# Sreyan88/audio-ssl

Hardware: AMD Instinct MI355X
Metric: upstream clips/sec (1s@16kHz, 64-mel) (higher is better)
Workload: dtype bf16; 1 GPU; delores-m upstream step (log-mel + 2 views + q/k conv encoders + MoCo + 3 Barlow heads + bwd + SGD), 1 s @ 16 kHz, 64 mel, batch 512/GPU, queue 65536; global_batch=512, parallelism=dp1

## Files before the change

audio-ssl_amd/src/engine.py:

```python
import os

import torch

from src import _native as N

import os as _os
_STEM_VALU = _os.environ.get("AUDIOSSL_STEM_VALU") == "1"
BN_MOMENTUM = 0.1
BN_EPS = 1e-5
_BN_FUSED = _os.environ.get("AUDIOSSL_BN_FUSED", "1") != "0"


ONE_STREAM = os.environ.get("AUDIOSSL_ONE_STREAM", "0") == "1"


_CAPTURE_ORIGIN = []


class capture_scope:

    def __enter__(self):
        _CAPTURE_ORIGIN.append(torch.cuda.current_stream())
        return self

# ... 462 lines not shown
    arg = _empty((Nimg, d), torch.uint8, like=H2)
    N.call("maxmean_fwd", dtype, int(y.dtype == torch.float32), H2, y, arg, Nimg, T3, d)
    return y, arg


def maxmean_backward(dtype, dy, arg, H2):
    Nimg, T3, d = H2.shape
    dA2 = _empty((Nimg * T3, d), N.torch_dtype(dtype), like=H2)
    N.call("maxmean_bwd", dtype, GD, dy, arg, H2, dA2, Nimg, T3, d)
    return dA2


class ProjCtx:
    pass


def projector_forward(PP, Y, dtype, groups, B, update_running=True, Wc=None):
    kin = Y.shape[1]
    c = ProjCtx()
    c.dtype, c.B, c.groups, c.kin, c.y = dtype, B, groups, kin, Y
    W = Wc if Wc is not None else tuple(cast(dtype, PP[f"projector.{i}.weight"]) for i in (0, 3, 6))
    c.W = W
    D = W[0].shape[0]
    c.D = D
    M = groups * B

    def bn(a, prefix, affine, relu, out, adt=None):
        g = PP[prefix + ".weight"] if affine else None
        b = PP[prefix + ".bias"] if affine else None
        return bn_train_apply(dtype, ad if adt is None else adt, a, B, D, g, b, PP[prefix + ".running_mean"], PP[prefix + ".running_var"],
                              update_running, groups, relu, out)
    td = N.torch_dtype(dtype)
    ad = _ad(dtype)
    c.ad = ad
    o32 = int(ad == N.F32)
    c.cmean = None
    if dtype == N.BF16 and Y.dtype == torch.float32 and not HP and B <= 1024 and kin % 32 == 0 and SYNC_BN is None:
        c.y_hi, c.cmean = center_cast(Y, groups, B)
        c.y_lo = None
        c.a1 = linear_fwd(dtype, c.y_hi, W[0], M, D, kin, out_f32=o32)
    elif dtype == N.BF16 and Y.dtype == torch.float32:
        c.y_hi, c.y_lo = _empty((M, kin), td, like=Y), _empty((M, kin), td, like=Y)
        N.call("split_bf16", Y, c.y_hi, c.y_lo, M * kin)
        c.a1 = torch.zeros(M, D, dtype=torch.float32, device=Y.device)
        gemm(dtype, 0, 0, M, D, kin, c.y_hi, kin, W[0], kin, c.a1, D, out_f32=1, atomic=1)
        gemm(dtype, 0, 0, M, D, kin, c.y_lo, kin, W[0], kin, c.a1, D, out_f32=1, atomic=1)
    else:
        c.y_hi, c.y_lo = Y, None
        c.a1 = linear_fwd(dtype, Y, W[0], M, D, kin, out_f32=o32)
    c.ad1 = N.F32 if c.a1.dtype == torch.float32 else ad
    c.h1 = _empty((M, D), td, like=Y)
    c.st1 = bn(c.a1, "projector.1", True, 1, c.h1, adt=c.ad1)
    if c.cmean is not None and update_running:
        N.call("shift_running_mean", W[0], c.cmean, PP["projector.1.running_mean"], D, kin, groups, BN_MOMENTUM)
    c.a2 = linear_fwd(dtype, c.h1, W[1], M, D, D, out_f32=o32)
    c.h2 = _empty((M, D), td, like=Y)
    c.st2 = bn(c.a2, "projector.4", True, 1, c.h2)
    c.z = linear_fwd(dtype, c.h2, W[2], M, D, D, out_f32=o32)
    c.zn = _empty((M, D), td, like=Y)
    c.st0 = bn(c.z, "bn", False, 0, c.zn)
    return c.zn, c


def projector_backward(c, PP, G, dzn, dy_rows=None):
    dtype, B, D, kin, groups = c.dtype, c.B, c.D, c.kin, c.groups
    M = groups * B
    td = N.torch_dtype(dtype)

    def bn_bwd(a, dh, st, relu, da, g_gamma, g_beta, adt=None):
        adt = c.ad if adt is None else adt
        """BatchNorm1d(train) backward per group (view).  SyncBatchNorm (`extras/delores-s/main.py:79` converts every BatchNorm of
        the model, the projector's included): the two means of the backward are over the GLOBAL batch of the view - this rank's
        sums are all-reduced between the statistics pass and the apply pass; the parameter gradients stay this rank's own sums
        (the data-parallel gradient all-reduce adds the ranks up afterwards)."""
        t = ARENA.scratch((2 * groups * D,), torch.float64, dzn)
        if SYNC_BN is None:
            N.call("colbn_bwd", dtype, adt, GD, a, dh, *st, relu, groups, B, D, t, da, g_gamma, g_beta)
            return
        N.call("colbn_bwd_stats", dtype, adt, GD, a, dh, *st, relu, groups, B, D, t)
        tg = SYNC_BN.all_reduce(t.clone())
        N.call("colbn_bwd_apply", dtype, adt, GD, a, dh, *st, relu, groups, B, D, tg, float(B * SYNC_BN.world), da)
        if g_gamma is not None:
            for g in range(groups):
                N.call("add_d2f", t[g * D:(g + 1) * D], g_beta, D)
                N.call("add_d2f", t[(groups + g) * D:(groups + g + 1) * D], g_gamma, D)
    dz = _empty((M, D), td, like=c.zn)
    bn_bwd(c.z, dzn, c.st0, 0, dz, None, None)
    linear_bwd_w(dtype, dz, c.h2, G["projector.6.weight"], M, D, D)
    dh2 = linear_bwd_x(dtype, dz, c.W[2], M, D, D, out_f32=1)
    da2 = _empty((M, D), td, like=c.zn)
    bn_bwd(c.a2, dh2, c.st2, 1, da2, G["projector.4.weight"], G["projector.4.bias"])
    linear_bwd_w(dtype, da2, c.h1, G["projector.3.weight"], M, D, D)
    dh1 = linear_bwd_x(dtype, da2, c.W[1], M, D, D, out_f32=1)
    da1 = _empty((M, D), td, like=c.zn)
    bn_bwd(c.a1, dh1, c.st1, 1, da1, G["projector.1.weight"], G["projector.1.bias"], adt=c.ad1)
    linear_bwd_w(dtype, da1, c.y_hi, G["projector.0.weight"], M, D, kin)
    if c.y_lo is not None:
        linear_bwd_w(dtype, da1, c.y_lo, G["projector.0.weight"], M, D, kin)
    rows = M if dy_rows is None else dy_rows
    if rows == 0:
        return None
    return linear_bwd_x(dtype, da1, c.W[0], rows, D, kin, out_f32=1)


def barlow_forward_backward(PP, G, Y, dtype, lambd, scale_loss, loss_out, need_dy1=True, need_dy2=True,
                            update_running=True, all_reduce=None, global_batch=None, backward=True, Wc=None):
    B = Y.shape[0] // 2
    zn, c = projector_forward(PP, Y, dtype, 2, B, update_running, Wc)
    D = c.D
    zn1, zn2 = zn[:B], zn[B:]
    denom = float(global_batch if global_batch else B)
    cmat = _empty((D, D), torch.float32, like=Y)
    gemm(dtype, 1, 1, D, D, B, zn1, D, zn2, D, cmat, D, alpha=1.0 / denom, out_f32=1)
    if all_reduce is not None:
        all_reduce(cmat)
    coef = (lambd if lambd else 1.0) * scale_loss
    dc = _empty((D, D), N.torch_dtype(dtype), like=Y)
    N.call("barlow_loss", dtype, cmat, D, coef, 2.0 * coef / denom, dc, loss_out)
    if not backward:
        return None
    dzn = _empty((2 * B, D), torch.float32, like=Y)
    gemm(dtype, 0, 0, B, D, D, zn2, D, dc, D, dzn[:B], D, out_f32=1)
    gemm(dtype, 0, 1, B, D, D, zn1, D, dc, D, dzn[B:], D, out_f32=1)
    rows = 2 * B if need_dy2 else (B if need_dy1 else 0)
    return projector_backward(c, PP, G, dzn, rows)


def _harr(ctype, xs):
    import ctypes
    vals = [x.data_ptr() if isinstance(x, torch.Tensor) else x for x in xs]
    return (ctype * len(vals))(*vals)


def _multi_check(*lists):
    for ts in lists:
        for t in ts:
            if t is not None and (not t.is_cuda or not t.is_contiguous()):
                raise RuntimeError("multi-problem launches need contiguous device tensors")


def gemm_multi(ta, tb, M, Nn, Ks, As, ldas, Bs, ldbs, Cs, ldc, alpha=1.0, out_f32=0, atomic=0, ksplit=1):
    import ctypes
    n = len(As)
    _multi_check(As, Bs, Cs)
    Ns = [Nn] * n if isinstance(Nn, int) else list(Nn)
    ldcs = [ldc] * n if isinstance(ldc, int) else list(ldc)
    adr = ctypes.addressof
    arrs = (_harr(ctypes.c_int, Ns), _harr(ctypes.c_int, Ks), _harr(ctypes.c_void_p, As), _harr(ctypes.c_long, ldas),
            _harr(ctypes.c_void_p, Bs), _harr(ctypes.c_long, ldbs), _harr(ctypes.c_void_p, Cs), _harr(ctypes.c_long, ldcs))
    N_, K_, A_, la_, B_, lb_, C_, lc_ = arrs
    if N.PROFILE is not None:
        N.PROFILE_NOTE = float(sum(2.0 * M * nn * kk for nn, kk in zip(Ns, Ks)))
    N.call("gemm_multi", n, ta, tb, M, adr(N_), adr(K_), float(alpha), adr(A_), adr(la_), adr(B_), adr(lb_), adr(C_), adr(lc_),
           out_f32, atomic, ksplit)


def gemm_multi_sgd(ta, tb, M, Nn, Ks, As, ldas, Bs, ldbs, Ps, Moms, Shadows, ldp, hyper, alpha=1.0):
    import ctypes
    n = len(As)
    _multi_check(As, Bs, Ps, Moms, [] if Shadows is None else Shadows)
    Ns = [Nn] * n if isinstance(Nn, int) else list(Nn)
    ldps = [ldp] * n if isinstance(ldp, int) else list(ldp)
    adr = ctypes.addressof
    vp = ctypes.c_void_p
    arrs = (_harr(ctypes.c_int, Ns), _harr(ctypes.c_int, Ks), _harr(vp, As), _harr(ctypes.c_long, ldas), _harr(vp, Bs),
            _harr(ctypes.c_long, ldbs), _harr(vp, Ps), _harr(vp, Moms), _harr(vp, Shadows if Shadows is not None else [None] * n),
            _harr(ctypes.c_long, ldps))
    if N.PROFILE is not None:
        N.PROFILE_NOTE = (float(sum(2.0 * M * nn * kk for nn, kk in zip(Ns, Ks))),
                          float(sum(2.0 * kk * (M + nn) + M * nn * (16.0 + (2.0 if Shadows is not None else 0.0)) for nn, kk in zip(Ns, Ks))))
    lr, mu, wd, gs, gs_dev = hyper
    N.call("gemm_multi_sgd", n, ta, tb, M, adr(arrs[0]), adr(arrs[1]), float(alpha), adr(arrs[2]), adr(arrs[3]), adr(arrs[4]), adr(arrs[5]),
           adr(arrs[6]), adr(arrs[7]), adr(arrs[8]), adr(arrs[9]), float(lr), float(mu), float(wd), float(gs), gs_dev)


def _heads_wgrad_split(D, kmax, M, nh):
    return _ksplit(D, kmax, M, max(256 // nh, 1))


def heads_wgrads_store(D, kins, M, grads_zero=True):
    nh = len(kins)
    return bool(grads_zero) and all(_heads_wgrad_split(D, k, M, nh) == 1 for k in (D, max(kins)))


def barlow_heads_forward_backward(PPs, Gs, Ys, dtype, lambds, scale_losses, loss_outs, update_running=True, backward=True,
                                  Wcs=None, grads_zero=False, dy_ready=None, sgd=None):
    import ctypes
    nh = len(Ys)
    B = Ys[0].shape[0] // 2
    M = 2 * B
    td = N.torch_dtype(dtype)
    dev = Ys[0].device
    W = Wcs if Wcs is not None else [tuple(cast(dtype, PP[f"projector.{i}.weight"]) for i in (0, 3, 6)) for PP in PPs]
    D = W[0][0].shape[0]
    kins = [Y.shape[1] for Y in Ys]
    ad = _ad(dtype)
    if dtype != N.BF16 or ad != N.BF16 or B > 1024 or D % 32:
        raise RuntimeError("grouped Barlow heads: bf16 path with B <= 1024 only")
    H = range(nh)
    vp, fl, adr = ctypes.c_void_p, ctypes.c_float, ctypes.addressof
    new = lambda rows, cols, t: [torch.empty(rows, cols, dtype=t, device=dev) for _ in H]

    def layer(xs, ws, ks, prefix, affine, relu):
        a = new(M, D, td)
        gemm_multi(0, 0, M, D, ks, xs, ks, ws, ks, a, D)
        out, st = new(M, D, td), new(4, 2 * D, torch.float32)
        par = lambda suffix, on=True: _harr(vp, [PP[prefix + suffix] if on else None for PP in PPs])
        arrs = (_harr(vp, a), par(".weight", affine), par(".bias", affine), par(".running_mean", update_running),
                par(".running_var", update_running), _harr(vp, out), _harr(vp, st))
        _multi_check(a, out, st)
        N.call("colbn_train_fwd_multi", nh, ad, adr(arrs[0]), adr(arrs[1]), adr(arrs[2]), adr(arrs[3]), adr(arrs[4]),
               BN_MOMENTUM, BN_EPS, relu, 2, B, D, adr(arrs[5]), adr(arrs[6]))
        return a, st, out
    ycs = [torch.empty(M, k, dtype=torch.bfloat16, device=dev) for k in kins]
    cms = [torch.empty(2, k, dtype=torch.float32, device=dev) for k in kins]
    _multi_check(list(Ys), ycs, cms)
    if any(Y.dtype != torch.float32 or k % 32 for Y, k in zip(Ys, kins)):
        raise RuntimeError("grouped Barlow heads: fp32 inputs with width % 32 == 0")
    arrs = (_harr(vp, list(Ys)), _harr(vp, ycs), _harr(vp, cms), _harr(ctypes.c_int, kins))
    N.call("center_cast_multi", nh, adr(arrs[0]), adr(arrs[1]), adr(arrs[2]), adr(arrs[3]), 2, B)
    a1, st1, h1 = layer(ycs, [W[h][0] for h in H], kins, "projector.1", True, 1)

    def shift_running():
        rms = [PP["projector.1.running_mean"] for PP in PPs]
        w0 = [W[h][0] for h in H]
        _multi_check(w0, rms)
        arrs = (_harr(vp, w0), _harr(vp, cms), _harr(vp, rms), _harr(ctypes.c_int, kins))
        N.call("shift_running_mean_multi", nh, adr(arrs[0]), adr(arrs[1]), adr(arrs[2]), D, adr(arrs[3]), 2, BN_MOMENTUM)
    shift_late = update_running and backward and dy_ready is not None
    if update_running and not shift_late:
        shift_running()
    a2, st2, h2 = layer(h1, [W[h][1] for h in H], [D] * nh, "projector.4", True, 1)
    z, st0, zn = layer(h2, [W[h][2] for h in H], [D] * nh, "bn", False, 0)
    dc = new(D, D, td)
    coefs = [(lambds[h] if lambds[h] else 1.0) * scale_losses[h] for h in H]
    dsc = [2.0 * c / B for c in coefs]
    if all(l.numel() == LOSS_REPLICAS for l in loss_outs) and D % 64 == 0:
        _multi_check([zn[h] for h in H], dc, list(loss_outs))
        arrs = (_harr(ctypes.c_int, [B] * nh), _harr(vp, [zn[h][:B] for h in H]), _harr(ctypes.c_long, [D] * nh),
                _harr(vp, [zn[h][B:] for h in H]), _harr(ctypes.c_long, [D] * nh), _harr(vp, dc), _harr(fl, coefs), _harr(fl, dsc),
                _harr(vp, list(loss_outs)))
        if N.PROFILE is not None:
            N.PROFILE_NOTE = float(nh * 2.0 * D * D * B)
        N.call("gemm_multi_barlow", nh, D, adr(arrs[0]), 1.0 / B, adr(arrs[1]), adr(arrs[2]), adr(arrs[3]), adr(arrs[4]), adr(arrs[5]),
               adr(arrs[6]), adr(arrs[7]), adr(arrs[8]))
    else:
        cm = new(D, D, torch.float32)
        gemm_multi(1, 1, D, D, [B] * nh, [zn[h][:B] for h in H], [D] * nh, [zn[h][B:] for h in H], [D] * nh, cm, D,
                   alpha=1.0 / B, out_f32=1)
        arrs = (_harr(vp, cm), _harr(fl, coefs), _harr(fl, dsc), _harr(vp, dc), _harr(vp, list(loss_outs)))
        _multi_check(list(loss_outs))
        N.call("barlow_loss_multi", nh, adr(arrs[0]), D, adr(arrs[1]), adr(arrs[2]), adr(arrs[3]), adr(arrs[4]))
    if not backward:
        return [None] * nh
    dzn = new(M, D, torch.float32)
    gemm_multi(0, 0, B, D, [D] * nh, [zn[h][B:] for h in H], [D] * nh, dc, [D] * nh, [dzn[h][:B] for h in H], D, out_f32=1)
    gemm_multi(0, 1, B, D, [D] * nh, [zn[h][:B] for h in H], [D] * nh, dc, [D] * nh, [dzn[h][B:] for h in H], D, out_f32=1)

    def bn_bwd(a, dh, st, relu, names):
        out = new(M, D, td)
        grads = lambda k: _harr(vp, [Gs[h][names[k]] if names else None for h in H])
        arrs = (_harr(vp, a), _harr(vp, dh), _harr(vp, st), _harr(vp, out), grads(0), grads(1))
        _multi_check(a, dh, st)
        N.call("colbn_bwd_multi", nh, ad, GD, adr(arrs[0]), adr(arrs[1]), adr(arrs[2]), relu, 2, B, D, adr(arrs[3]),
               adr(arrs[4]), adr(arrs[5]))
        return out

    def wgrad(dys, xs, name, ks):
        split = _heads_wgrad_split(D, max(ks), M, nh)
        if sgd is not None:
            if split != 1 or Wcs is None:
                raise RuntimeError("fused SGD needs unsplit weight gradients and the flat weight shadows")
            li = {"projector.0.weight": 0, "projector.3.weight": 1, "projector.6.weight": 2}[name]
            gemm_multi_sgd(1, 1, D, ks, [M] * nh, dys, [D] * nh, xs, ks, [PPs[h][name] for h in H], [sgd["momentum"][h][name] for h in H],
                           [W[h][li] for h in H], ks, sgd["hyper"])
            return
        gemm_multi(1, 1, D, ks, [M] * nh, dys, [D] * nh, xs, ks, [Gs[h][name] for h in H], ks, out_f32=1,
                   atomic=1 if split > 1 else (0 if grads_zero else 2), ksplit=split)

    def dgrad(dys, ws, Ks, rows):
        out = [torch.empty(rows, k, dtype=torch.float32, device=dev) for k in Ks]
        gemm_multi(0, 1, rows, Ks, [D] * nh, [dy[:rows] for dy in dys], [D] * nh, ws, Ks, out, Ks, out_f32=1)
        return out
    later = []
    defer = (lambda fn: later.append(fn)) if dy_ready is not None else (lambda fn: fn())
    dz = bn_bwd(z, dzn, st0, 0, None)
    defer(lambda: wgrad(dz, h2, "projector.6.weight", [D] * nh))
    dh2 = dgrad(dz, [W[h][2] for h in H], [D] * nh, M)
    da2 = bn_bwd(a2, dh2, st2, 1, ("projector.4.weight", "projector.4.bias"))
    defer(lambda: wgrad(da2, h1, "projector.3.weight", [D] * nh))
    dh1 = dgrad(da2, [W[h][1] for h in H], [D] * nh, M)
    da1 = bn_bwd(a1, dh1, st1, 1, ("projector.1.weight", "projector.1.bias"))
    defer(lambda: wgrad(da1, ycs, "projector.0.weight", kins))
    dy = dgrad(da1, [W[h][0] for h in H], kins, B)
    if dy_ready is not None:
        dy_ready()
    if shift_late:
        shift_running()
    for fn in later:
        fn()
    return dy


def moco_forward_backward(dtype, q, k, queue, queue_shadow, temperature, loss_out, backward=True):
    B, dim = q.shape
    K = queue.shape[1]
    td = N.torch_dtype(dtype)
    qn, kn = _empty((B, dim), td, like=q), _empty((B, dim), td, like=q)
    qn32, kn32 = _empty((B, dim), torch.float32, like=q), _empty((B, dim), torch.float32, like=q)
    qinv, kinv = _empty((B,), torch.float32, like=q), _empty((B,), torch.float32, like=q)
    lpos = _empty((B,), torch.float32, like=q)
    N.call("moco_prep", dtype, q, k, B, dim, 1.0 / temperature, qn, qn32, qinv, kn, kn32, kinv, lpos)
    lse = _empty((B,), torch.float32, like=q)
    dlpos = _empty((B,), torch.float32, like=q)
    Pm = None
    if dtype == N.BF16 and K % 8 == 0 and dim % 8 == 0:
        nslot = (K + 63) // 64
        part = _empty((B, nslot, 2), torch.float32, like=q)
        N.call("moco_logits", 1, qn, queue_shadow, B, K, dim, 1.0 / temperature, part, None, 0.0, None)
        N.call("moco_lse_merge", lpos, part, B, nslot, 1.0 / (B * temperature), lse, loss_out, dlpos)
        if not backward:
            return None, kn32
        Pm = _empty((B, K), td, like=q)
        N.call("moco_logits", 2, qn, queue_shadow, B, K, dim, 1.0 / temperature, None, lse, 1.0 / (B * temperature), Pm)
    else:
        lneg = _empty((B, K), torch.float32, like=q)
        gemm(dtype, 0, 1, B, K, dim, qn, dim, queue_shadow, K, lneg, K, alpha=1.0 / temperature, out_f32=1)
        N.call("moco_ce_fwd", lpos, lneg, B, K, lse, loss_out)
        if not backward:
            return None, kn32
        Pm = _empty((B, K), td, like=q)
        N.call("moco_ce_bwd", dtype, lpos, lneg, lse, B, K, 1.0 / (B * temperature), Pm, dlpos)
    dqn = ARENA.zeros((B, dim), torch.float32, device=q.device)
    gemm(dtype, 0, 0, B, dim, K, Pm, K, queue_shadow, K, dqn, dim, out_f32=1, atomic=1, ksplit=_ksplit(B, dim, K, 256))
    dq = _empty((B, dim), td, like=q)
    N.call("l2norm_bwd", dtype, dqn, dlpos, kn32, qn32, qinv, B, dim, dq)
    return dq, kn32
```

include/audiossl_hip.h:

```cpp
#ifndef AUDIOSSL_HIP_H
#define AUDIOSSL_HIP_H

#include <stdint.h>

#ifdef __cplusplus
extern "C" {
#endif

#define AUDIOSSL_OK 0
#define AUDIOSSL_EINVAL (-1)
#define AUDIOSSL_ELAUNCH (-2)
#define AUDIOSSL_EALIGN (-3)

int audiossl_logmel_fwd(const float* wave, float* out, int B, int L, int T, int n_fft, int hop, int n_mels, int taps,
                        const float* win, const float* tw, const float* melw, const int* mel_start, float eps_pow,
                        float eps_log, int apply_log, void* stream);

int audiossl_clip_moments(const float* x, double* mom, int B, int n, void* stream);
int audiossl_runnorm_scan(const double* mom, int B, int n_elem, long long* state_i, float* state_f, float* mu_out,
                          float* sd_out, void* stream);
int audiossl_aug_normalize(const float* x, const float* mu, const float* sd, float* bank, long slot0, int R, int B, int n,
                           void* stream);
int audiossl_aug_views(const float* bank, int R, const int* ip, const float* fp, float* out1, float* out2, int B, int F,
                       int T, int canvas_h, int canvas_w, int log_mix, void* stream);
int audiossl_aug_plan_host(uint32_t* np_key, int* np_pos, uint32_t* py_key, int* py_pos, int B, int F, int T,
                           long long clips_seen, long long* n_entries, int R, int n_memory, int use_mix, double ratio,
                           int use_rrc, double fs_lo, double fs_hi, double ts_lo, double ts_hi, int canvas_h,
                           int canvas_w, int use_spec, int spec_F, int spec_T, int spec_nf, int spec_nt, const int* lens,
                           int unit, int* starts, int* ip, float* fp, int* masks);

int audiossl_resample_sinc(const float* x, float* y, int clips, int n_orig, int n_out, const int* n, const int* off_l,
                           const int* off_r, const double* eta_l, const double* eta_r, const double* win, const double* delta,
                           int nwin, int index_step, void* stream);

int audiossl_kmix_cluster(const float* views, const float* centroids, int n_views, int F, int T, int K, int* cluster,
                          void* stream);
int audiossl_kmix_apply(const float* views, const float* ring, const int* slot, const float* coef, int n_views, int n,
                        int log_mix, float* out, void* stream);
int audiossl_mask_fill(float* x, const int* tab, int n_img, int max_masks, int F, int T, int zero_fill, void* stream);

int audiossl_conv1_stats(const float* img, int N, int F, int T, const float* w, const float* bias, const float* gamma,
                         const float* beta, float* running_mean, float* running_var, float momentum, float eps,
                         double* mom, float* scale, float* shift, float* save_mean, float* save_rstd, void* stream);
#define AUDIOSSL_CONV1_XL_PARTS 4
int audiossl_conv1_fwd(int dtype, const float* img, int N, int F, int T, const float* w, const float* bias,
                       const float* scale, const float* shift, void* out, float* xl, void* stream);
int audiossl_conv1_bwd(int dtype, int conv_dtype, const float* img, int N, int F, int T, const float* w, const float* bias,
                       const float* gamma, const float* scale, const float* shift, const float* mean, const float* rstd,
                       const double* mom, const void* dP, const void* dxl, float* acc, float* dW, float* dbias,
                       float* dgamma, float* dbeta, void* stream);

int audiossl_colstats(int dtype, const void* x, int groups, long M, int C, long ld, int want_sq, double* sum,
                      double* sumsq, void* stream);
int audiossl_bn_finalize(const double* sum, const double* sumsq, int groups, double count, int C, const float* gamma,
                         const float* beta, float* running_mean, float* running_var, float momentum, float eps,
                         float* scale, float* shift, float* save_mean, float* save_rstd, void* stream);
int audiossl_bn_relu_pool_fwd(int dtype, int ydtype, const void* Y, const float* scale, const float* shift, void* P, int N,
                              int Ti, int Fi, void* stream);
int audiossl_bn_relu_pool_train_fwd(int dtype, int ydtype, const void* Y, const double* sum, const double* sumsq, int stat_replicas,
                                    double count, const float* gamma, const float* beta, float* running_mean, float* running_var,
                                    float momentum, float eps, void* P, float* scale, float* shift, float* save_mean, float* save_rstd,
                                    int N, int Ti, int Fi, void* stream);
int audiossl_tmean_fwd(int dtype, int out_f32, const void* P, void* xl, int N, int To, int Fo, void* stream);
int audiossl_tmean3_fwd(int dtype, int out_f32, const void* P1, void* x1, const float* x1_parts, int To1, int Fo1, const void* P2,
                        void* x2, int To2, int Fo2, const void* P3, void* x3, int To3, int Fo3, int N, void* stream);
int audiossl_bn_relu_pool_bwd(int dtype, int ydtype, int gdtype, const void* Y, const void* dP, const void* dxl, const float* scale,
                              const float* shift, const float* mean, const float* rstd, float* stat, void* dY,
                              float* dgamma, float* dbeta, int N, int Ti, int Fi, void* stream);
int audiossl_bn_relu_pool_bwd_p(int dtype, int ydtype, int gdtype, const void* Y, const void* P, const void* dP, const void* dxl,
                                const float* scale, const float* shift, const float* mean, const float* rstd, float* stat, void* dY,
                                float* dgamma, float* dbeta, int N, int Ti, int Fi, void* stream);
int audiossl_conv1_moments(const float* img, int N, int F, int T, double* mom, void* stream);
int audiossl_conv1_finalize(double* mom_totals, const float* w, const float* bias, const float* gamma, const float* beta,
                            float* running_mean, float* running_var, float momentum, float eps, double count, float* scale,
                            float* shift, float* save_mean, float* save_rstd, void* stream);
int audiossl_conv1_bwd_sums(int dtype, int conv_dtype, const float* img, int N, int F, int T, const float* w, const float* bias,
                            const float* gamma, const float* scale, const float* shift, const float* mean, const float* rstd,
                            const double* mom, const void* dP, const void* dxl, float* acc, float* lstat, void* stream);
int audiossl_conv1_bwd_finalize(const float* acc, const double* mom, const float* w, const float* bias, const float* gamma,
                                const float* mean, const float* rstd, double count_global, const float* gstat, float* dW,
                                float* dbias, float* dgamma, float* dbeta, void* stream);
int audiossl_bn_relu_pool_bwd_stats(int dtype, int ydtype, int gdtype, const void* Y, const void* dP, const void* dxl,
                                    const float* scale, const float* shift, const float* mean, const float* rstd, float* stat,
                                    int N, int Ti, int Fi, void* stream);
int audiossl_bn_relu_pool_bwd_apply(int dtype, int ydtype, int gdtype, const void* Y, const void* dP, const void* dxl,
                                    const float* scale, const float* shift, const float* mean, const float* rstd, float* stat,
                                    const float* gstat, double count_global, void* dY, float* dgamma, float* dbeta, int N, int Ti,
                                    int Fi, void* stream);
int audiossl_colbn_bwd_stats(int dtype, int adtype, int gdtype, const void* a, const void* dh, const float* scale,
                             const float* shift, const float* mean, const float* rstd, int relu, int groups, long M, int C,
                             double* tmp, void* stream);
int audiossl_colbn_bwd_apply(int dtype, int adtype, int gdtype, const void* a, const void* dh, const float* scale,
                             const float* shift, const float* mean, const float* rstd, int relu, int groups, long M, int C,
                             const double* sums, double count, void* da, void* stream);
int audiossl_im2col3x3(int dtype, const void* X, void* col, int N, int Ti, int Fi, void* stream);
int audiossl_pack_conv_w(int dtype, const float* W, void* Wf, void* Wd, void* stream);
int audiossl_pack_conv_w2(int dtype, const float* Wa, void* Wfa, void* Wda, const float* Wb, void* Wfb, void* Wdb, void* stream);
int audiossl_unpack_conv_dw(const float* dWp, float* dW, void* stream);

int audiossl_conv3x3_fwd(const void* X, const void* W, const float* bias, void* Y, int out_f32, double* sum,
                         double* sumsq, int stat_replicas, int N, int Ti, int Fi, void* stream);
int audiossl_conv3x3_wgrad(const void* dY, const void* X, float* dWp, float* workspace, long workspace_floats, int N, int Ti,
                           int Fi, void* stream);

int audiossl_gemm(int dtype, int trans_a, int trans_b, int M, int N, int K, float alpha, const void* A, long lda,
                  const void* B, long ldb, void* C, long ldc, const float* bias, int relu, const uint8_t* keep, long ldk,
                  float keep_scale, const void* gate, long ldg, int out_f32, int atomic, int ksplit, const float* resid,
                  long ldr, void* stream);

int audiossl_gemm_dropout(int trans_a, int trans_b, int M, int N, int K, float alpha, const void* A, long lda, const void* B,
                          long ldb, void* C, long ldc, const float* bias, int relu, unsigned long long seed, float p,
                          const long long* counter, float keep_scale, void* stream);

int audiossl_gemm_multi(int count, int trans_a, int trans_b, int M, const int* N, const int* K, float alpha,
                        const void* const* A, const long* lda, const void* const* B, const long* ldb, void* const* C,
                        const long* ldc, int out_f32, int atomic, int ksplit, void* stream);
int audiossl_gemm_multi_sgd(int count, int trans_a, int trans_b, int M, const int* Nv, const int* K, float alpha,
                            const void* const* A, const long* lda, const void* const* B, const long* ldb, float* const* P,
                            float* const* Mom, void* const* Shadow, const long* ldp, float lr, float momentum, float weight_decay,
                            float grad_scale, const float* grad_scale_dev, void* stream);
int audiossl_gemm_multi_barlow(int count, int D, const int* K, float alpha, const void* const* A, const long* lda,
                               const void* const* B, const long* ldb, void* const* dc, const float* coef, const float* dscale,
                               float* const* loss_rep, void* stream);

int audiossl_maxmean_fwd(int dtype, int out_f32, const void* H, void* y, uint8_t* arg, int N, int Tt, int D, void* stream);
int audiossl_maxmean_bwd(int dtype, int gdtype, const void* dy, const uint8_t* arg, const void* H, void* dA, int N, int Tt,
                         int D, void* stream);

int audiossl_colbn_fwd(int dtype, int adtype, const void* a, const float* scale, const float* shift, int relu, void* h,
                       int groups, long M, int C, void* stream);
int audiossl_colbn_train_fwd(int dtype, int adtype, const void* a, const float* gamma, const float* beta,
                             float* running_mean, float* running_var, float momentum, float eps, int relu, int groups,
                             long M, int C, void* h, float* scale, float* shift, float* save_mean, float* save_rstd,
                             void* stream);
int audiossl_colbn_bwd(int dtype, int adtype, int gdtype, const void* a, const void* dh, const float* scale, const float* shift, const float* mean,
                       const float* rstd, int relu, int groups, long M, int C, double* tmp, void* da, float* dgamma,
                       float* dbeta, void* stream);
int audiossl_colbn_train_fwd_multi(int count, int adtype, const void* const* a, const float* const* gamma,
                                   const float* const* beta, float* const* running_mean, float* const* running_var,
                                   float momentum, float eps, int relu, int groups, long M, int C, void* const* h,
                                   float* const* stats, void* stream);
int audiossl_colbn_bwd_multi(int count, int adtype, int gdtype, const void* const* a, const void* const* dh,
                             const float* const* stats, int relu, int groups, long M, int C, void* const* da,
                             float* const* dgamma, float* const* dbeta, void* stream);
int audiossl_barlow_loss_multi(int count, const float* const* c, int D, const float* coef, const float* dscale,
                               void* const* dc, float* const* loss_out, void* stream);
int audiossl_add_d2f(const double* src, float* dst, int n, void* stream);
int audiossl_barlow_loss(int dtype, const float* c, int D, float coef, float dscale, void* dc, float* loss_out,
                         void* stream);

int audiossl_l2norm_fwd(int dtype, const float* q, int B, int D, void* qn, float* qn32, float* inv_norm, void* stream);
int audiossl_moco_prep(int dtype, const float* q, const float* k, int B, int D, float scale, void* qn, float* qn32, float* qinv,
                       void* kn, float* kn32, float* kinv, float* lpos, void* stream);
int audiossl_rowdot(const float* a, const float* b, int B, int D, float scale, float* out, void* stream);
int audiossl_moco_ce_fwd(const float* lpos, const float* lneg, int B, int K, float* lse, float* loss_out, void* stream);
int audiossl_moco_ce_bwd(int dtype, const float* lpos, const float* lneg, const float* lse, int B, int K, float gscale,
                         void* P, float* dlpos, void* stream);
int audiossl_moco_logits(int mode, const void* qn, const void* queue, int B, int K, int dim, float inv_t, float* part,
                         const float* lse, float gscale, void* P, void* stream);
int audiossl_moco_lse_merge(const float* lpos, const float* part, int B, int nslot, float gscale, float* lse,
                            float* loss_out, float* dlpos, void* stream);
int audiossl_l2norm_bwd(int dtype, const float* dqn, const float* dlpos, const float* kn32, const float* qn32,
                        const float* inv_norm, int B, int D, void* dq, void* stream);
int audiossl_enqueue(int dtype, const float* keys, int B, int D, int K, int ptr, long long* ptr_dev, float* queue, void* shadow,
                     void* stream);
int audiossl_ema_update(float* pk, const float* pq, long n, float m, void* shadow, void* stream);

int audiossl_set_prezeroed(int on);
int audiossl_last_kernel(char* name, int capacity);

int audiossl_sgd_momentum(float* p, float* g, float* buf, long n, float lr, float momentum, float weight_decay,
                          int first, float grad_scale, const float* grad_scale_dev, void* shadow_bf16, int zero_grad,
                          void* stream);
int audiossl_sgd_momentum_segments(float* p, float* g, float* buf, const long* segs, int nseg, long max_n, float lr, float momentum,
                                   float weight_decay, int first, float grad_scale, const float* grad_scale_dev, void* shadow_bf16,
                                   int zero_grad, void* stream);
int audiossl_zero_segments(float* g, const long* segs, int nseg, long max_n, void* stream);
int audiossl_cast(int dtype, const float* src, void* dst, long n, void* stream);
int audiossl_cast_back(int dtype, const void* src, float* dst, long n, void* stream);
int audiossl_dropout_mask(uint8_t* keep, long n, unsigned long long seed, float p, const long long* counter, void* stream);
int audiossl_relu_bwd(int dtype, const void* g, const void* h, void* out, long n, void* stream);
int audiossl_bn_eval_affine(const float* gamma, const float* beta, const float* running_mean, const float* running_var,
                            float eps, int C, float* scale, float* shift, void* stream);
int audiossl_axpy(float* y, const float* x, float a, long n, void* stream);
int audiossl_split_bf16(const float* x, void* hi, void* lo, long n, void* stream);
int audiossl_center_cast(const float* y, void* yc, float* cmean, int groups, long M, int C, void* stream);
int audiossl_shift_running_mean(const void* W, const float* cmean, float* running_mean, int D, int K, int groups,
                                float momentum, void* stream);
int audiossl_center_cast_multi(int count, const float* const* y, void* const* yc, float* const* cmean, const int* C, int groups,
                               long M, void* stream);
int audiossl_shift_running_mean_multi(int count, const void* const* W, const float* const* cmean, float* const* running_mean,
                                      int D, const int* K, int groups, float momentum, void* stream);

int audiossl_ntxent_fwd(const float* sim, int N, int B, float* lse, float* loss_out, void* stream);
int audiossl_ntxent_bwd(int dtype, const float* sim, const float* lse, int N, int B, float gscale, void* dsim, void* stream);

int audiossl_row_argmax(const float* dot, long N, int K, long long* assign, void* stream);
int audiossl_kmeans_accumulate(const float* x, const long long* assign, long N, int K, int D, float* sums, int* counts,
                               void* stream);
int audiossl_kmeans_update(const float* sums, const int* counts, int K, int D, float* centroids, void* stream);
int audiossl_kmeans_update_mean(const float* sums, const int* counts, int K, int D, float* centroids, void* stream);
int audiossl_row_sqnorm(const float* x, int rows, int D, float scale, float* out, void* stream);
int audiossl_ce_rows(int dtype, const float* logits, const long long* target, int B, int K, int ignore_index, int* cnt,
                     float* loss_out, void* dlogits, void* stream);

int audiossl_softmax_rows_fwd(const float* x, float* y, int M, int C, void* stream);
int audiossl_softmax_rows_bwd(const float* y, const float* gy, float* gx, int M, int C, void* stream);

int audiossl_attn_fwd(const void* qkv, void* out, float* lse, int B, int S, int H, float scale, void* stream);
int audiossl_attn_bwd(const void* qkv, const void* out, const void* dout, const float* lse, void* dqkv, int B, int S, int H,
                      float scale, void* stream);
int audiossl_layernorm_fwd(const float* x, const float* gamma, const float* beta, void* y, float* y32, float* mean, float* rstd,
                           int M, int C, float eps, void* stream);
int audiossl_layernorm_bwd(const float* dy, const float* x, const float* mean, const float* rstd, const float* gamma,
                           float* dres, float* dgamma, float* dbeta, int M, int C, void* stream);
int audiossl_gelu_fwd(const void* a, void* h, long n, void* stream);
int audiossl_gelu_bwd(const void* a, const void* dh, void* da, long n, void* stream);
int audiossl_patch_unfold(const float* x, void* out, int B, int F, int T, int fstride, int tstride, void* stream);
int audiossl_tile_rows(const float* src, float* out, long rows, int period, int group, float scale, int C, void* stream);
int audiossl_adamw(float* p, const float* g, float* m, float* v, long n, float lr, float beta1, float beta2, float eps,
                   float weight_decay, float grad_scale, const long long* step, void* stream);

int audiossl_mvit_pool_fwd(const void* qkv, int ldq, int col0, const float* w, const float* gamma, const float* beta, float* out,
                           float* z, float* mean, float* rstd, int B, int heads, int d, int H, int W, int Ho, int Wo, int sh, int sw,
                           float eps, void* stream);
int audiossl_mvit_pool_bwd(const void* qkv, int ldq, int col0, const float* w, const float* gamma, const float* dout, const float* z,
                           const float* mean, const float* rstd, float* dz, float* dw, float* dgamma, float* dbeta, void* dqkv, int B,
                           int heads, int d, int H, int W, int Ho, int Wo, int sh, int sw, void* stream);
int audiossl_mvit_attn_fwd(const float* q, const float* k, const float* v, const float* rh, const float* rw, const int* ih,
                           const int* iw, void* out, float* lse, int B, int heads, int d, int qh, int qw, int kh, int kw, int nrh,
                           int nrw, int residual, float scale, void* stream);
int audiossl_mvit_attn_bwd(const float* q, const float* k, const float* v, const float* rh, const float* rw, const int* ih,
                           const int* iw, const void* dout, const float* lse, float* dq, float* dk, float* dv, float* drh, float* drw,
                           int B, int heads, int d, int qh, int qw, int kh, int kw, int nrh, int nrw, int residual, float scale,
                           void* stream);
int audiossl_tokpool_max_fwd(const float* x, float* y, void* arg, int B, int H, int W, int C, int kh, int kw, int sh, int sw,
                             void* stream);
int audiossl_tokpool_max_bwd(const float* dy, const void* arg, float* dx, int B, int H, int W, int C, int kh, int kw, int sh, int sw,
                             void* stream);

int audiossl_lars_step(float* p, const float* g, float* mu, const void* seg, int n_seg, const float* lr, float weight_decay,
                       float momentum, float eta, float grad_scale, double* norms, void* stream);
int audiossl_larc_step(float* p, const float* g, float* mu, const void* seg, int n_seg, float lr, float weight_decay,
                       float momentum, float trust_coefficient, float eps, int clip, float grad_scale, double* norms,
                       void* stream);

#ifdef __cplusplus
}
#endif
#endif
```

Before: 269,600 clips/s.

## Fuse MoCo InfoNCE forward/backward into flash-style split-K kernel with merge

Replaces the two-pass MoCo logits path (logits→LSE merge→recompute probabilities into a BxK matrix→GEMM for dq→l2norm backward) with a single flash-attention-style kernel. It computes the online softmax and accumulates P·queue per key slice, followed by a merge kernel that combines slices, computes lse, loss, dlpos and applies the l2-norm backward to produce dq. This avoids materializing the BxK probability matrix and the extra pass over the queue. In exchange it writes per-slice partial outputs of size nslice×B×dim, rounds probabilities to bf16 before the MFMA, and is restricted to dim==128.

```diff
diff --git a/audio-ssl_amd/csrc/moco.hip b/audio-ssl_amd/csrc/moco.hip
--- /dev/null
+++ b/audio-ssl_amd/csrc/moco.hip
@@ -0,0 +1,223 @@
+#include "common.h"
+
+namespace {
+
+constexpr int KT = 128;
+constexpr int QB = 128;
+typedef __attribute__((address_space(3))) bf16x4* lds4_t;
+
+__device__ __forceinline__ int img_off(int d, int u) { return d * 256 + 8 * (u ^ (((d & 3) << 3) | ((d >> 2) & 7))); }
+__device__ __forceinline__ int row_of(int r, int half) { return (r & 3) + 8 * (r >> 2) + 4 * half; }
+
+template <int DIM>
+__global__ __launch_bounds__(256) void moco_infonce_kernel(const bf16* __restrict__ qn, const bf16* __restrict__ queue, int B,
+                                                           int K, int nslice, int slice_len, int nrb, float inv_t,
+                                                           float* __restrict__ part_o, float* __restrict__ part_ml) {
+    extern __shared__ __attribute__((aligned(16))) unsigned char smem[];
+    constexpr int TILE_BYTES = KT * DIM * 2;
+    constexpr int NLD = DIM * (KT / 8) / 256;
+    constexpr int KB = 4;
+    const int L = blockIdx.x, qq = L >> 3;
+    const int slice = (L & 7) + 8 * (qq / nrb), rb = qq % nrb;
+    if (slice >= nslice) return;
+    const int tid = threadIdx.x, lane = tid & 63, w = tid >> 6, h = lane >> 5, l31 = lane & 31;
+    const int k_begin = slice * slice_len, k_end = min(K, k_begin + slice_len);
+    const int ntiles = (k_end - k_begin + KT - 1) / KT;
+    const int q = rb * QB + w * 32 + l31;
+    bf16x8 fq[DIM / 16];
+#pragma unroll
+    for (int ds = 0; ds < DIM / 16; ++ds) fq[ds] = q < B ? Vec8<bf16>::load(qn + (long)q * DIM + 16 * ds + 8 * h).v : Vec8<bf16>::zero().v;
+
+    bf16x8 st[NLD];
+    auto load_tile = [&](int k0) {
+#pragma unroll
+        for (int v = 0; v < NLD; ++v) {
+            const int idx = tid + 256 * v, d = idx >> 4, key = k0 + 8 * (idx & 15);
+            st[v] = key < k_end ? Vec8<bf16>::load(queue + (long)d * K + key).v : Vec8<bf16>::zero().v;
+        }
+    };
+    auto store_tile = [&](unsigned char* img) {
+#pragma unroll
+        for (int v = 0; v < NLD; ++v) {
+            const int idx = tid + 256 * v, d = idx >> 4, c = idx & 15;
+            const int f = ((d & 3) << 3) | ((d >> 2) & 7);
+            bf16x8 x = st[v];
+            if (f & 1) x = bf16x8{x[4], x[5], x[6], x[7], x[0], x[1], x[2], x[3]};
+            *reinterpret_cast<bf16x8*>(img + d * 256 + 16 * (c ^ (f >> 1))) = x;
+        }
+    };
+
+    f32x16 o[DIM / 32];
+#pragma unroll
+    for (int dt = 0; dt < DIM / 32; ++dt)
+#pragma unroll
+        for (int r = 0; r < 16; ++r) o[dt][r] = 0.f;
+    float m = -3.0e38f, l = 0.f;
+    load_tile(k_begin);
+    store_tile(smem);
+    __syncthreads();
+    const int q4 = (lane & 15) >> 2, p4 = lane & 3, g16 = (lane >> 4) & 1;
+    for (int t = 0; t < ntiles; ++t) {
+        const int k0 = k_begin + t * KT;
+        const unsigned char* img = smem + (t & 1) * TILE_BYTES;
+        if (t + 1 < ntiles) load_tile(k0 + KT);
+
+#pragma unroll
+        for (int hb = 0; hb < 4 / KB; ++hb) {
+            f32x16 s[KB];
+#pragma unroll
+            for (int kb = 0; kb < KB; ++kb) {
+#pragma unroll
+                for (int r = 0; r < 16; ++r) s[kb][r] = 0.f;
+                const int u = (hb * KB + kb) * 8 + 4 * g16 + p4;
+#pragma unroll
+                for (int ds = 0; ds < DIM / 16; ++ds) {
+                    const int d0 = 16 * ds + 8 * h + q4;
+                    const bf16x4 a0 = __builtin_amdgcn_ds_read_tr16_b64_v4bf16((lds4_t)(img + img_off(d0, u)));
+                    const bf16x4 a1 = __builtin_amdgcn_ds_read_tr16_b64_v4bf16((lds4_t)(img + img_off(d0 + 4, u)));
+                    const bf16x8 a = bf16x8{a0[0], a0[1], a0[2], a0[3], a1[0], a1[1], a1[2], a1[3]};
+                    s[kb] = __builtin_amdgcn_mfma_f32_32x32x16_bf16(a, fq[ds], s[kb], 0, 0, 0);
+                }
+            }
+            const int kk = k0 + 32 * KB * hb;
+            const bool tail = kk + 32 * KB > k_end;
+            float tm = -3.0e38f;
+#pragma unroll
+            for (int kb = 0; kb < KB; ++kb)
+#pragma unroll
+                for (int r = 0; r < 16; ++r) {
+                    float x = s[kb][r] * inv_t;
+                    if (tail && kk + 32 * kb + row_of(r, h) >= k_end) x = -3.0e38f;
+                    s[kb][r] = x;
+                    tm = fmaxf(tm, x);
+                }
+            tm = fmaxf(tm, __shfl_xor(tm, 32, 64));
+            const float mn = fmaxf(m, tm), alpha = __expf(m - mn);
+            m = mn;
+            l *= alpha;
+#pragma unroll
+            for (int dt = 0; dt < DIM / 32; ++dt)
+#pragma unroll
+                for (int r = 0; r < 16; ++r) o[dt][r] *= alpha;
+#pragma unroll
+            for (int kb = 0; kb < KB; ++kb)
+#pragma unroll
+                for (int r = 0; r < 16; ++r) {
+                    const float p = __expf(s[kb][r] - mn);
+                    s[kb][r] = p;
+                    l += p;
+                }
+#pragma unroll
+            for (int kb = 0; kb < KB; ++kb)
+#pragma unroll
+                for (int st2 = 0; st2 < 2; ++st2) {
+                    bf16x8 pb;
+#pragma unroll
+                    for (int j = 0; j < 8; ++j) pb[j] = (bf16)s[kb][8 * st2 + j];
+                    const int u = (hb * KB + kb) * 8 + 4 * st2 + h;
+#pragma unroll
+                    for (int dt = 0; dt < DIM / 32; ++dt) {
+                        const int d = dt * 32 + l31;
+                        const bf16x4 a0 = *reinterpret_cast<const bf16x4*>(img + img_off(d, u));
+                        const bf16x4 a1 = *reinterpret_cast<const bf16x4*>(img + img_off(d, u + 2));
+                        const bf16x8 a = bf16x8{a0[0], a0[1], a0[2], a0[3], a1[0], a1[1], a1[2], a1[3]};
+                        o[dt] = __builtin_amdgcn_mfma_f32_32x32x16_bf16(a, pb, o[dt], 0, 0, 0);
+                    }
+                }
+        }
+        if (t + 1 < ntiles) store_tile(smem + ((t + 1) & 1) * TILE_BYTES);
+        __syncthreads();
+    }
+    l += __shfl_xor(l, 32, 64);
+    if (q < B) {
+        float* po = part_o + ((long)slice * B + q) * DIM;
+#pragma unroll
+        for (int dt = 0; dt < DIM / 32; ++dt)
+#pragma unroll
+            for (int g = 0; g < 4; ++g)
+                *reinterpret_cast<f32x4*>(po + dt * 32 + 8 * g + 4 * h) = f32x4{o[dt][4 * g], o[dt][4 * g + 1], o[dt][4 * g + 2], o[dt][4 * g + 3]};
+        if (h == 0) *reinterpret_cast<float2*>(part_ml + ((long)slice * B + q) * 2) = make_float2(m, l);
+    }
+}
+
+template <int DIM>
+__global__ __launch_bounds__(256) void moco_infonce_merge_kernel(const float* __restrict__ part_o, const float* __restrict__ part_ml,
+                                                                 int B, int nslice, const float* __restrict__ lpos,
+                                                                 const float* __restrict__ kn32, const float* __restrict__ qn32,
+                                                                 const float* __restrict__ qinv, float inv_B, float gscale,
+                                                                 float* __restrict__ lse_out, float* __restrict__ loss_out,
+                                                                 float* __restrict__ dlpos_out, bf16* __restrict__ dq) {
+    static_assert(DIM * 2 == 256, "two threads per column");
+    extern __shared__ float wsh[];
+    __shared__ float sh[16], half_sum[DIM];
+    const long b = blockIdx.x;
+    const int tid = threadIdx.x, d = tid % DIM, hf = tid / DIM;
+    const float lp = lpos[b];
+    float M = lp;
+    for (int s = tid; s < nslice; s += 256) M = fmaxf(M, part_ml[((long)s * B + b) * 2]);
+    M = wave_max(M);
+    __syncthreads();
+    if ((tid & 63) == 0) sh[tid >> 6] = M;
+    __syncthreads();
+    M = fmaxf(fmaxf(sh[0], sh[1]), fmaxf(sh[2], sh[3]));
+    float Ls = 0.f;
+    for (int s = tid; s < nslice; s += 256) {
+        const float2 ml = *reinterpret_cast<const float2*>(part_ml + ((long)s * B + b) * 2);
+        Ls += ml.y * __expf(ml.x - M);
+    }
+    Ls = block_sum(Ls, sh) + __expf(lp - M);
+    const float lse = M + logf(Ls);
+    const float dl = (expf(lp - lse) - 1.f) * gscale;
+    for (int s = tid; s < nslice; s += 256) wsh[s] = __expf(part_ml[((long)s * B + b) * 2] - lse);
+    __syncthreads();
+    float acc = 0.f;
+#pragma unroll 8
+    for (int s = hf; s < nslice; s += 2) acc += wsh[s] * part_o[((long)s * B + b) * DIM + d];
+    if (hf == 1) half_sum[d] = acc;
+    __syncthreads();
+    const float g = (acc + half_sum[d]) * gscale + dl * kn32[b * DIM + d];
+    const float qv = qn32[b * DIM + d];
+    const float sdot = block_sum(hf == 0 ? qv * g : 0.f, sh);
+    if (hf == 0) dq[b * DIM + d] = (bf16)((g - qv * sdot) * qinv[b]);
+    if (tid == 0) {
+        lse_out[b] = lse;
+        dlpos_out[b] = dl;
+        atomicAdd(loss_out, (lse - lp) * inv_B);
+    }
+}
+
+template <int DIM>
+int launch_infonce(const bf16* qn, const bf16* queue, int B, int K, int slice_len, float inv_t, const float* lpos, const float* kn32,
+                   const float* qn32, const float* qinv, float gscale, float* part, float* lse, float* loss_out, float* dlpos, bf16* dq,
+                   hipStream_t s) {
+    const size_t lds = 2 * KT * DIM * 2;
+    static bool lds_set = false;
+    if (!lds_set) {
+        if (hipFuncSetAttribute(reinterpret_cast<const void*>(&moco_infonce_kernel<DIM>), hipFuncAttributeMaxDynamicSharedMemorySize,
+                                (int)lds) != hipSuccess) return ASSL_ELAUNCH;
+        lds_set = true;
+    }
+    const int nslice = ceil_div(K, slice_len), nrb = ceil_div(B, QB);
+    float* part_o = part;
+    float* part_ml = part + (long)nslice * B * DIM;
+    hipLaunchKernelGGL(moco_infonce_kernel<DIM>, dim3(ceil_div(nslice, 8) * 8 * nrb), dim3(256), lds, s, qn, queue, B, K, nslice, slice_len,
+                       nrb, inv_t, part_o, part_ml);
+    if (hipGetLastError() != hipSuccess) return ASSL_ELAUNCH;
+    hipLaunchKernelGGL(moco_infonce_merge_kernel<DIM>, dim3(B), dim3(256), nslice * sizeof(float), s, part_o, part_ml, B, nslice, lpos,
+                       kn32, qn32, qinv,
+                       1.f / (float)B, gscale, lse, loss_out, dlpos, dq);
+    ASSL_LAUNCH_CHECK();
+}
+
+}
+
+extern "C" int audiossl_moco_infonce(const void* qn, const void* queue, int B, int K, int dim, int slice_len, float inv_t,
+                                     const float* lpos, const float* kn32, const float* qn32, const float* qinv, float gscale,
+                                     float* part, long part_floats, float* lse, float* loss_out, float* dlpos, void* dq, void* stream) {
+    ASSL_REQUIRE(qn && queue && lpos && kn32 && qn32 && qinv && part && lse && loss_out && dlpos && dq);
+    ASSL_REQUIRE(B > 0 && K > 0 && K % 8 == 0 && dim == 128 && slice_len > 0 && slice_len % KT == 0);
+    ASSL_REQUIRE(ceil_div(K, slice_len) <= 8192 && part_floats >= (long)ceil_div(K, slice_len) * B * (dim + 2));
+    if (!ASSL_ALIGNED16(qn) || !ASSL_ALIGNED16(queue) || !ASSL_ALIGNED16(part)) return ASSL_EALIGN;
+    return launch_infonce<128>((const bf16*)qn, (const bf16*)queue, B, K, slice_len, inv_t, lpos, kn32, qn32, qinv, gscale, part, lse,
+                               loss_out, dlpos, (bf16*)dq, (hipStream_t)stream);
+}
diff --git a/audio-ssl_amd/src/engine.py b/audio-ssl_amd/src/engine.py
--- a/audio-ssl_amd/src/engine.py
+++ b/audio-ssl_amd/src/engine.py
@@ -788,6 +788,16 @@
     return dy
 
 
+_MOCO_FUSED = os.environ.get("AUDIOSSL_MOCO_FUSED", "1") != "0"
+
+
+def _moco_slice_len(B, K):
+    sl = 1024
+    while sl > 128 and ((B + 127) // 128) * ((K + sl - 1) // sl) < 256:
+        sl //= 2
+    return sl
+
+
 def moco_forward_backward(dtype, q, k, queue, queue_shadow, temperature, loss_out, backward=True):
     B, dim = q.shape
     K = queue.shape[1]
@@ -800,6 +810,14 @@
     lse = _empty((B,), torch.float32, like=q)
     dlpos = _empty((B,), torch.float32, like=q)
     Pm = None
+    if backward and _MOCO_FUSED and dtype == N.BF16 and K % 8 == 0 and dim == 128:
+        sl = _moco_slice_len(B, K)
+        nsl = (K + sl - 1) // sl
+        part = _empty((nsl * B * (dim + 2),), torch.float32, like=q)
+        dq = _empty((B, dim), td, like=q)
+        N.call("moco_infonce", qn, queue_shadow, B, K, dim, sl, 1.0 / temperature, lpos, kn32, qn32, qinv,
+               1.0 / (B * temperature), part, part.numel(), lse, loss_out, dlpos, dq)
+        return dq, kn32
     if dtype == N.BF16 and K % 8 == 0 and dim % 8 == 0:
         nslot = (K + 63) // 64
         part = _empty((B, nslot, 2), torch.float32, like=q)
diff --git a/include/audiossl_hip.h b/include/audiossl_hip.h
--- a/include/audiossl_hip.h
+++ b/include/audiossl_hip.h
@@ -162,6 +162,9 @@
                             float* loss_out, float* dlpos, void* stream);
 int audiossl_l2norm_bwd(int dtype, const float* dqn, const float* dlpos, const float* kn32, const float* qn32,
                         const float* inv_norm, int B, int D, void* dq, void* stream);
+int audiossl_moco_infonce(const void* qn, const void* queue, int B, int K, int dim, int slice_len, float inv_t, const float* lpos,
+                          const float* kn32, const float* qn32, const float* qinv, float gscale, float* part, long part_floats,
+                          float* lse, float* loss_out, float* dlpos, void* dq, void* stream);
 int audiossl_enqueue(int dtype, const float* keys, int B, int D, int K, int ptr, long long* ptr_dev, float* queue, void* shadow,
                      void* stream);
 int audiossl_ema_update(float* pk, const float* pq, long n, float m, void* shadow, void* stream);
```

After: 271,800 clips/s, median of 6. Within noise of the previous version (+0.8%).
